# LDeakin/VkVolume

Hardware: AMD Instinct MI355X
Metric: Mray/s (higher is better)
Workload: dtype f32

## Files before the change

### vkvolume_amd/csrc/ray_setup.hpp

```cpp
#pragma once

#include "raymarch_args.hpp"
#include "volume_sampling.hpp"

template <int SKIP, bool FAST>
__device__ __forceinline__ bool ray_setup_impl(const RayMarchArgs &A, uint32_t px, uint32_t py, Ray &R, bool &ok)
{
	R.r = R.g = R.b = R.a = 0.0f;
	R.depth = 0.0f;
	R.n_vol = R.n_dist = R.n_empty = 0;
	R.n_steps = 0, R.i = 0, R.i_min = 0, R.first_hit = 0, R.ul = 0;
	R.fragment = false;
	const int W = A.W, H = A.H, D = A.D;

	const float fx = (float) px + 0.5f, fy = (float) py + 0.5f;
	float       dx = __builtin_fmaf(fy, A.ddy[0], __builtin_fmaf(fx, A.ddx[0], A.dir00[0]));
	float       dy = __builtin_fmaf(fy, A.ddy[1], __builtin_fmaf(fx, A.ddx[1], A.dir00[1]));
	float       dz = __builtin_fmaf(fy, A.ddy[2], __builtin_fmaf(fx, A.ddx[2], A.dir00[2]));
	{
		const float len = __builtin_sqrtf(__builtin_fmaf(dz, dz, __builtin_fmaf(dy, dy, dx * dx)));
		if (FAST)
		{
			ok = ok && div_ordinary(len) && div_ordinary_num(dx) && div_ordinary_num(dy) && div_ordinary_num(dz);
			const float r = recip_refined(len);
			dx = div_by(dx, len, r), dy = div_by(dy, len, r), dz = div_by(dz, len, r);
		}
		else
			dx /= len, dy /= len, dz /= len;
	}
	const float ox = A.cam[0], oy = A.cam[1], oz = A.cam[2];
	float       t_near = -INFINITY, t_far = INFINITY;
	bool        miss   = false;
	{
		const float dv[3] = {dx, dy, dz}, ov[3] = {ox, oy, oz};
#pragma unroll
		for (int a = 0; a < 3; ++a)
		{
			if (dv[a] == 0.0f)
			{
				if (ov[a] < 0.0f || ov[a] > 1.0f)
					miss = true;
			}
			else
			{
				float inv;
				if (FAST)
				{
					ok  = ok && div_ordinary(dv[a]);
					inv = recip_exact(dv[a]);
				}
				else
					inv = 1.0f / dv[a];
				const float ta = (0.0f - ov[a]) * inv, tb = (1.0f - ov[a]) * inv;
				t_near = g_max(t_near, g_min(ta, tb));
				t_far  = g_min(t_far, g_max(ta, tb));
			}
		}
	}
	if (miss)
		return false;
	const float Ap = __builtin_fmaf(A.plane_tex[2], oz, __builtin_fmaf(A.plane_tex[1], oy, A.plane_tex[0] * ox)) + A.plane_tex[3];
	const float Bp = __builtin_fmaf(A.plane_tex[2], dz, __builtin_fmaf(A.plane_tex[1], dy, A.plane_tex[0] * dx));
	if (!(Bp > 0.0f))
		return false;
	float t_plane;
	if (FAST)
	{
		ok      = ok && div_ordinary(Bp) && div_ordinary_num(0.0f - Ap);
		t_plane = div_by(0.0f - Ap, Bp, recip_refined(Bp));
	}
	else
		t_plane = (0.0f - Ap) / Bp;
	const float t0      = g_max(t_near, t_plane);
	if (!(t0 < t_far))
		return false;
	const float ex = __builtin_fmaf(t0, dx, ox), ey = __builtin_fmaf(t0, dy, oy), ez = __builtin_fmaf(t0, dz, oz);
	R.fragment = true;

	float frag_depth = 0.0f, frag_depth_front = 0.0f, position[4] = {0, 0, 0, 0};
	if (A.depth_attachment)
	{
		const float pm[4] = {ex - 0.5f, ey - 0.5f, ez - 0.5f, 1.0f};
		float       a4[4], b4[4];
		mat4_mul_vec4(A.model, pm, a4);
		mat4_mul_vec4(A.view, a4, b4);
		mat4_mul_vec4(A.proj, b4, position);
		frag_depth       = A.in_depth[R.o];
		frag_depth_front = position[2] / position[3];
		if (frag_depth > frag_depth_front)
		{
			R.fragment = false;
			return false;
		}
		R.depth = frag_depth;
	}

	float rdx, rdy, rdz;
	{
		const float vx = ex - ox, vy = ey - oy, vz = ez - oz;
		const float len = __builtin_sqrtf(__builtin_fmaf(vz, vz, __builtin_fmaf(vy, vy, vx * vx)));
		if (FAST)
		{
			ok = ok && div_ordinary(len) && div_ordinary_num(vx) && div_ordinary_num(vy) && div_ordinary_num(vz);
			const float r = recip_refined(len);
			rdx = div_by(vx, len, r), rdy = div_by(vy, len, r), rdz = div_by(vz, len, r);
		}
		else
			rdx = vx / len, rdy = vy / len, rdz = vz / len;
	}
	float xx, xy, xz, ray_distance;
	{
		float ix, iy, iz;
		if (FAST)
		{
			ok = ok && div_ordinary(rdx) && div_ordinary(rdy) && div_ordinary(rdz);
			ix = recip_exact(rdx), iy = recip_exact(rdy), iz = recip_exact(rdz);
		}
		else
			ix = 1.0f / rdx, iy = 1.0f / rdy, iz = 1.0f / rdz;
		const float tminx = -ex * ix, tminy = -ey * iy, tminz = -ez * iz;
		const float tmaxx = (1.0f - ex) * ix, tmaxy = (1.0f - ey) * iy, tmaxz = (1.0f - ez) * iz;
		const float t2x = g_max(tminx, tmaxx), t2y = g_max(tminy, tmaxy), t2z = g_max(tminz, tmaxz);
		const float tFar = g_min(g_min(t2x, t2y), t2z);
		xx = __builtin_fmaf(tFar, rdx, ex), xy = __builtin_fmaf(tFar, rdy, ey), xz = __builtin_fmaf(tFar, rdz, ez);
		const float vx = ex - xx, vy = ey - xy, vz = ez - xz;
		ray_distance = __builtin_sqrtf(__builtin_fmaf(vz, vz, __builtin_fmaf(vy, vy, vx * vx)));
	}
	if (A.depth_attachment)
	{
		const float clip[4] = {(position[0] * frag_depth) / frag_depth_front, (position[1] * frag_depth) / frag_depth_front,
		                       (position[2] * frag_depth) / frag_depth_front, position[3]};
		float       w4[4], m4[4];
		mat4_mul_vec4(A.view_proj_inv, clip, w4);
		w4[0] /= w4[3], w4[1] /= w4[3], w4[2] /= w4[3], w4[3] /= w4[3];
		mat4_mul_vec4(A.model_inv, w4, m4);
		const float ix = m4[0] + 0.5f, iy = m4[1] + 0.5f, iz = m4[2] + 0.5f;
		const float vx = ex - ix, vy = ey - iy, vz = ez - iz;
		const float dd = __builtin_sqrtf(__builtin_fmaf(vz, vz, __builtin_fmaf(vy, vy, vx * vx)));
		if (dd < ray_distance)
		{
			xx = ix, xy = iy, xz = iz;
			ray_distance = dd;
		}
	}
	if (A.test == VKV_TEST_RAY_ENTRY)
	{
		R.r = ex, R.g = ey, R.b = ez, R.a = 1.0f;
		return false;
	}
	if (A.test == VKV_TEST_RAY_EXIT)
	{
		R.r = xx, R.g = xy, R.b = xz, R.a = 1.0f;
		return false;
	}

	const int   dim_max = max(max(W, H), D);
	const float nf      = __builtin_ceilf((float) dim_max * ray_distance * A.sampling_factor);
	if (!(nf >= 2.0f && nf <= 16777216.0f))
		return false;
	float sx, sy, sz;
	{
		const float den = nf - 1.0f, nx = rdx * ray_distance, ny = rdy * ray_distance, nz = rdz * ray_distance;
		if (FAST)
		{
			ok = ok && div_ordinary_num(nx) && div_ordinary_num(ny) && div_ordinary_num(nz);
			const float r = recip_refined(den);
			sx = div_by(nx, den, r), sy = div_by(ny, den, r), sz = div_by(nz, den, r);
		}
		else
			sx = nx / den, sy = ny / den, sz = nz / den;
	}
	{
		const float qx = ex + sx, qy = ey + sy, qz = ez + sz;
		if (qx <= 0.0f || qy <= 0.0f || qz <= 0.0f || qx >= 1.0f || qy >= 1.0f || qz >= 1.0f)
			return false;
	}
	R.ex = ex, R.ey = ey, R.ez = ez, R.sx = sx, R.sy = sy, R.sz = sz;
	R.n_steps = (int) nf;

	R.six = R.siy = R.siz = 0.0f;
	R.dmap                = nullptr;
	if (SKIP != VKV_SKIP_NONE)
	{
		if (FAST)
		{
			const float nx = sx * (float) W, ny = sy * (float) H, nz = sz * (float) D;
			ok = ok && div_ordinary(A.block_size[0]) && div_ordinary(A.block_size[1]) && div_ordinary(A.block_size[2]) && div_ordinary_num(nx) &&
			     div_ordinary_num(ny) && div_ordinary_num(nz);
			const float tx = div_by(nx, A.block_size[0], recip_refined(A.block_size[0]));
			const float ty = div_by(ny, A.block_size[1], recip_refined(A.block_size[1]));
			const float tz = div_by(nz, A.block_size[2], recip_refined(A.block_size[2]));
			ok    = ok && div_ordinary(tx) && div_ordinary(ty) && div_ordinary(tz);
			R.six = recip_exact(tx), R.siy = recip_exact(ty), R.siz = recip_exact(tz);
		}
		else
		{
			R.six = 1.0f / ((sx * (float) W) / A.block_size[0]);
			R.siy = 1.0f / ((sy * (float) H) / A.block_size[1]);
			R.siz = 1.0f / ((sz * (float) D) / A.block_size[2]);
		}
		if (SKIP == VKV_SKIP_ANISOTROPIC_DISTANCE)
			R.dmap = A.maps[(rdz < 0 ? 1 : 0) + (rdy < 0 ? 2 : 0) + (rdx < 0 ? 4 : 0)];
		else
			R.dmap = A.maps[0];
	}
	R.i = 0, R.i_min = 0, R.ulx = R.uly = R.ulz = 0, R.ul = 0;
	R.occupied  = true;
	R.first_hit = R.n_steps;
	return true;
}

template <int SKIP>
__device__ __forceinline__ bool ray_setup(const RayMarchArgs &A, uint32_t px, uint32_t py, Ray &R)
{
	bool       ok      = true;
	const bool marched = ray_setup_impl<SKIP, true>(A, px, py, R, ok);
	if (__builtin_amdgcn_ballot_w64(!ok) == 0ull)
		return marched;
	bool unused = true;
	return ray_setup_impl<SKIP, false>(A, px, py, R, unused);
}

__device__ __forceinline__ void ray_clear(Ray &R)
{
	R.r = R.g = R.b = R.a = 0.0f;
	R.depth = 0.0f;
	R.n_vol = R.n_dist = R.n_empty = 0;
	R.n_steps = 0, R.i = 0, R.i_min = 0, R.first_hit = 0, R.ul = 0;
	R.fragment = false;
}

__device__ __forceinline__ void ray_finish(const RayMarchArgs &A, Ray &R, bool marched)
{
	if (marched)
	{
		if (A.out_depth && R.a > 0.0f && R.first_hit < R.n_steps)
		{
			const float fi   = (float) R.first_hit;
			const float p[4] = {__builtin_fmaf(fi, R.sx, R.ex) - 0.5f, __builtin_fmaf(fi, R.sy, R.ey) - 0.5f, __builtin_fmaf(fi, R.sz, R.ez) - 0.5f, 1.0f};
			float       a4[4], b4[4], c4[4];
			mat4_mul_vec4(A.model, p, a4);
			mat4_mul_vec4(A.view, a4, b4);
			mat4_mul_vec4(A.proj, b4, c4);
			R.depth = c4[2] / c4[3];
		}
		if (A.test == VKV_TEST_NUM_TEXTURE_SAMPLES)
		{
			const int      dim_max     = max(max(A.W, A.H), A.D);
			const uint32_t n_steps_max = (uint32_t) (__builtin_ceilf((float) dim_max * __builtin_sqrtf(3.0f)) * A.sampling_factor);
			const float    v           = (float) (R.n_vol + R.n_dist) / (float) n_steps_max;
			R.r = R.g = R.b = v;
			R.a             = 1.0f;
		}
	}
	const size_t o = R.o;
	if (!R.fragment)
	{
		if (A.blend)
		{
			if (A.out_counts)
				A.out_counts[o * 3 + 0] = A.out_counts[o * 3 + 1] = A.out_counts[o * 3 + 2] = 0;
			return;
		}
		if (A.depth_attachment)
			R.depth = A.in_depth[o];
		if (A.out_color)
			store_float4_nt(A.out_color, o, 0.0f, 0.0f, 0.0f, 0.0f);
		if (A.out_rgba8)
			__builtin_nontemporal_store(0u, reinterpret_cast<uint32_t *>(A.out_rgba8) + o);
		if (A.out_counts)
			A.out_counts[o * 3 + 0] = A.out_counts[o * 3 + 1] = A.out_counts[o * 3 + 2] = 0;
		if (A.out_depth)
			__builtin_nontemporal_store(R.depth, A.out_depth + o);
		return;
	}
	else if (A.blend)
	{
		const float om = 1.0f - R.a;
		if (A.out_color)
		{
			float4 d = reinterpret_cast<float4 *>(A.out_color)[o];
			d.x = __builtin_fmaf(om, d.x, R.r), d.y = __builtin_fmaf(om, d.y, R.g), d.z = __builtin_fmaf(om, d.z, R.b), d.w = R.a * om;
			reinterpret_cast<float4 *>(A.out_color)[o] = d;
		}
		if (A.out_rgba8)
		{
			const uint32_t d = reinterpret_cast<uint32_t *>(A.out_rgba8)[o];
			const float    r = __builtin_fmaf(om, unorm8(d & 255u), R.r), g = __builtin_fmaf(om, unorm8((d >> 8) & 255u), R.g),
			            b = __builtin_fmaf(om, unorm8((d >> 16) & 255u), R.b);
			reinterpret_cast<uint32_t *>(A.out_rgba8)[o] = (uint32_t) quantise_rgba8(r) | ((uint32_t) quantise_rgba8(g) << 8) |
			                                               ((uint32_t) quantise_rgba8(b) << 16) | ((uint32_t) quantise_rgba8(R.a * om) << 24);
		}
		if (A.out_counts)
		{
			A.out_counts[o * 3 + 0] = R.n_vol;
			A.out_counts[o * 3 + 1] = R.n_dist;
			A.out_counts[o * 3 + 2] = R.n_empty;
		}
		if (A.out_depth)
			A.out_depth[o] = R.depth;
		return;
	}
// ... 43 lines not shown
```

### vkvolume_amd/csrc/raymarch.hip

```cpp
#include <algorithm>
#include <cmath>
#include <cstdio>
#include <cstdlib>
#include <cstring>
#include <mutex>
#include <new>
#include <vector>

#include "raymarch_inst.hpp"
#include "launchers.hpp"
#include "render_args.hpp"

constexpr int kCostBins = 1024;

__device__ __forceinline__ void tile_order_from_cost(uint32_t *__restrict__ cost, uint32_t *__restrict__ order_out, uint32_t count)
{
	__shared__ uint32_t s_bin[kCostBins];
	constexpr int       kPerThread = 40;
	for (int b = threadIdx.x; b < kCostBins; b += blockDim.x)
		s_bin[b] = 0;
	__syncthreads();
	for (uint32_t base = 0; base < count; base += 256u * kPerThread)
	{
		uint32_t c[kPerThread];
// ... 190 lines not shown
	{
		const double pn = std::sqrt((double) plane_tex[0] * plane_tex[0] + (double) plane_tex[1] * plane_tex[1] + (double) plane_tex[2] * plane_tex[2]);
		if (!std::isfinite(pn) || !(pn > 0.0) || !std::isfinite((double) plane_tex[3]))
			clip = false;
		for (int c = 0; c < 8 && clip; ++c)
			sd[c] = (double) plane_tex[0] * (c & 1) + (double) plane_tex[1] * ((c >> 1) & 1) + (double) plane_tex[2] * ((c >> 2) & 1) + (double) plane_tex[3] + 1e-4 * pn;
	}
	for (int c = 0; c < 8; ++c)
		if (!clip || sd[c] >= 0.0)
			vert[n_vert][0] = (double) (c & 1), vert[n_vert][1] = (double) ((c >> 1) & 1), vert[n_vert][2] = (double) ((c >> 2) & 1), ++n_vert;
	if (clip)
		for (int c = 0; c < 8; ++c)
			for (int axis = 0; axis < 3; ++axis)
			{
				const int d = c | (1 << axis);
				if (d == c || (sd[c] >= 0.0) == (sd[d] >= 0.0))
					continue;
				const double u = sd[c] / (sd[c] - sd[d]);
				for (int k = 0; k < 3; ++k)
					vert[n_vert][k] = (double) ((c >> k) & 1) + u * ((double) ((d >> k) & 1) - (double) ((c >> k) & 1));
				++n_vert;
			}
	if (n_vert == 0)
		return kScreenBoundEmpty;
	double lo_x = 1e300, hi_x = -1e300, lo_y = 1e300, hi_y = -1e300;
	for (int i = 0; i < n_vert; ++i)
	{
		const double v[3] = {vert[i][0] - cam[0], vert[i][1] - cam[1], vert[i][2] - cam[2]};
		const double fa = (inv[0][0] * v[0] + inv[0][1] * v[1] + inv[0][2] * v[2]) / det, fb = (inv[1][0] * v[0] + inv[1][1] * v[1] + inv[1][2] * v[2]) / det;
		const double g  = (inv[2][0] * v[0] + inv[2][1] * v[1] + inv[2][2] * v[2]) / det;
		if (!(g > 1e-6) || !std::isfinite(fa) || !std::isfinite(fb))
			return kScreenBoundNone;
		lo_x = std::min(lo_x, fa / g), hi_x = std::max(hi_x, fa / g), lo_y = std::min(lo_y, fb / g), hi_y = std::max(hi_y, fb / g);
	}
	out[0] = std::floor(lo_x - 0.5) - 2.0, out[1] = std::ceil(hi_x - 0.5) + 2.0, out[2] = std::floor(lo_y - 0.5) - 2.0, out[3] = std::ceil(hi_y - 0.5) + 2.0;
	if (out[1] < 0.0 || out[3] < 0.0 || out[0] > 4.0e9 || out[2] > 4.0e9)
		return kScreenBoundEmpty;
	return kScreenBoundRect;
}

static void screen_bound_of_box(RayMarchArgs &a, const VkvTuning &T)
{
	a.cull_x0 = 0u, a.cull_x1 = ~0u, a.cull_y0 = 0u, a.cull_y1 = ~0u;
	if (!T.screen_cull)
		return;
	double    b[4];
	const int kind = screen_bound(a.cam, a.dir00, a.ddx, a.ddy, a.plane_tex, b);
	if (kind == kScreenBoundNone)
		return;
	if (kind == kScreenBoundEmpty)
	{
		a.cull_x0 = 1u, a.cull_x1 = 0u;
		return;
	}
	a.cull_x0 = b[0] <= 0.0 ? 0u : (uint32_t) b[0], a.cull_y0 = b[2] <= 0.0 ? 0u : (uint32_t) b[2];
	a.cull_x1 = b[1] >= 4.0e9 ? ~0u : (uint32_t) b[1], a.cull_y1 = b[3] >= 4.0e9 ? ~0u : (uint32_t) b[3];
}

void screen_tile_rect(const VkvRayCastUniform *rc, const VkvRayGen *rg, uint32_t iw, uint32_t ih, uint32_t tw, uint32_t th, uint32_t align, VkvTileRect *out)
{
	const uint32_t tiles_x = (iw + tw - 1) / tw, tiles_y = (ih + th - 1) / th;
	*out = VkvTileRect{0u, 0u, tiles_x, tiles_y};
	double    b[4];
	const int kind = screen_bound(rc->camera_pos_tex, rg->dir00, rg->ddx, rg->ddy, rc->plane_tex, b);
	if (kind == kScreenBoundNone)
		return;
	if (kind == kScreenBoundEmpty || b[0] >= (double) iw || b[2] >= (double) ih)
	{
		*out = VkvTileRect{0u, 0u, 1u, 1u};
		return;
	}
	const uint32_t x0 = b[0] <= 0.0 ? 0u : (uint32_t) b[0], y0 = b[2] <= 0.0 ? 0u : (uint32_t) b[2];
	const uint32_t x1 = b[1] >= (double) (iw - 1) ? iw - 1 : (uint32_t) b[1], y1 = b[3] >= (double) (ih - 1) ? ih - 1 : (uint32_t) b[3];
	const uint32_t q = align > 1 ? align : 1u;
	uint32_t       tx0 = (x0 / tw) / q * q, ty0 = (y0 / th) / q * q;
	uint32_t       tx1 = std::min(tiles_x, (x1 / tw + q) / q * q), ty1 = std::min(tiles_y, (y1 / th + q) / q * q);
	*out = VkvTileRect{tx0, ty0, tx1 - tx0, ty1 - ty0};
}

int fill_render_args(vkv_ctx *ctx, const VkvRenderParams *P, const float *alpha_lut, RayMarchArgs &a, hipStream_t s, const VkvTuning &T, bool setup, bool batch)
{
	bool whole_schedule = fill_shared_args(P, a);
	for (int i = 0; i < 3; ++i)
		a.block_size[i] = P->ray_cast.block_size[i];
	a.grad_modifier = P->transfer_function.grad_magnitude_modifier;
	a.grad = P->d_gradient, a.tf = P->d_transfer_function;
	a.tf_bits = P->d_transfer_function_bits;
	for (int i = 0; i < 8; ++i)
		a.maps[i] = P->d_distance_maps[i];
	a.in_depth = P->d_in_depth;
	a.blend    = P->blend_over_target != 0;
	a.fill_rgba8_rows = (a.out_rgba8 && !a.out_color && !a.out_counts && !a.out_depth && !a.blend && (a.img_w & 3u) == 0 && (((uintptr_t) a.out_rgba8) & 15u) == 0) ? 1u : 0u;
	{
		const VkvTileRect &r = P->tiles.rect;
		const uint32_t     full_x = (a.img_w + a.tile_w - 1) / a.tile_w, full_y = (a.img_h + a.tile_h - 1) / a.tile_h;
		a.fill_tiles = 0, a.img_tiles_x = full_x, a.rect_tx0 = a.rect_ty0 = a.rect_th = 0;
		if (!whole_schedule && P->tiles.fill_outside)
		{
			if (!batch || T.scheduler == 1 || T.batch_mode == 1 || (uint64_t) full_x * full_y - (uint64_t) r.w * r.h > (uint64_t) kFillPerTile * r.w * r.h)
			{
				whole_schedule = true;
				a.tile_count = full_x * full_y, a.tiles_x = full_x, a.org_x = a.org_y = 0u;
			}
			else
				a.fill_tiles = full_x * full_y - r.w * r.h, a.rect_tx0 = r.x0, a.rect_ty0 = r.y0, a.rect_th = r.h;
		}
	}
	const uint64_t nb   = (uint64_t) a.blocks_per_tile * a.tile_count;
	a.nblocks           = 0;
	if (nb == 0)
		return VKV_OK;
	if (nb > 0x3fffffffull)
		return set_error(ctx, VKV_E_UNSUPPORTED, "render: too many tiles for one launch");
	if ((uint64_t) a.img_w * a.img_h > 0xffffffffull / 4 || nb * 256 > 0xffffffffull / 4)
		return set_error(ctx, VKV_E_UNSUPPORTED, "render: frame too large for one launch");
	a.nblocks     = (uint32_t) nb;
	a.test        = P->options.test;
	a.queue_heads = nullptr;
	a.tile_cost = nullptr, a.order_out = nullptr;
	a.trace       = reinterpret_cast<unsigned long long *>(ctx->d_trace);
	a.back        = (int) std::ceil(P->transfer_function.sampling_factor);
	a.clamp_always = T.clamp_always != 0 ? 1u : 0u;
	a.wave_pw_log2 = T.wave_shape == 4 ? 2u : (T.wave_shape == 8 ? 3u : (T.wave_shape == 16 ? 4u : wave_patch_log2(a.ddx, a.ddy, a.W, a.H, a.D)));
	{
		const float m[3] = {(float) a.mw, (float) a.mh, (float) a.md};
		for (int k = 0; k < 3; ++k)
			a.mapf[k] = m[k], a.mapb[k] = std::nextafterf(m[k], 0.0f);
	}
	a.addr_lut = nullptr, a.lut_y = a.lut_z = a.lut_words = a.lut_full = 0;
	if (a.packed && T.address_tables != 0)
		a.addr_lut = packed_addr_lut(ctx, a.W, a.H, a.D, &a.lut_y, &a.lut_z, &a.lut_words, &a.lut_full, s, setup);
	screen_bound_of_box(a, T);
	a.tile_order = (T.tile_order_linear || !whole_schedule) ? nullptr
	                                                         : tile_start_order(ctx, a.img_w, a.img_h, a.tile_w, a.tile_h, a.tile_first, a.tile_stride, a.tile_count, s, setup);
	a.order_h = 0;
	if (!whole_schedule && !T.tile_order_linear && a.tile_first == 0 && a.tile_stride == 1 && (uint64_t) a.tile_count == (uint64_t) a.tiles_x * P->tiles.rect.h)
		a.order_h = P->tiles.rect.h;
	for (int i = 0; i < 256; ++i)
		a.alpha_lut[i] = alpha_lut[i];
	return VKV_OK;
}

static bool apply_feedback(vkv_ctx *ctx, RayMarchArgs &a, hipStream_t s)
{
	(void) s;
	const void *      target = a.out_rgba8 ? (const void *) a.out_rgba8 : (const void *) a.out_color;
	vkv_ctx::TileFeedback *     f = nullptr;
	std::lock_guard<std::mutex> lock(ctx->mutex);
	const uint32_t              period = ctx->tuning.feedback_period < 1u ? 1u : ctx->tuning.feedback_period;
	if (!ctx->tuning.feedback || !target || a.tile_count < 64 || ctx->d_debug_orders)
		return false;
	for (auto *e : ctx->feedback)
		if (e->target == target && e->img_w == a.img_w && e->img_h == a.img_h && e->tile_w == a.tile_w && e->tile_h == a.tile_h && e->first == a.tile_first &&
		    e->stride == a.tile_stride && e->count == a.tile_count && e->org_x == a.org_x && e->org_y == a.org_y && e->tiles_x == a.tiles_x)
		{
			f = e;
			break;
		}
	if (!f)
		return false;
	float dir[3], len2 = 0.0f;
	for (int i = 0; i < 3; ++i)
	{
		dir[i] = a.dir00[i] + 0.5f * ((float) a.img_w * a.ddx[i] + (float) a.img_h * a.ddy[i]);
		len2 += dir[i] * dir[i];
	}
	const float inv = len2 > 0.0f ? 1.0f / std::sqrt(len2) : 0.0f;
// ... 258 lines not shown
```

### vkvolume_amd/csrc/raymarch_args.hpp

```cpp
#pragma once

#include <stdint.h>

constexpr int kTraceWords = 10;
constexpr uint32_t kFillPerTile = 3;

struct RayMarchArgs
{
	float dir00[3], ddx[3], ddy[3];
	float cam[3];
	float plane_tex[4];
	float block_size[3];
	float model[16], view[16], proj[16];
	float view_proj_inv[16], model_inv[16];
	float sampling_factor, grad_modifier;
	int W, H, D, mw, mh, md;
	const uint8_t * vol, *grad, *tf;
	const uint8_t * packed;
	int             pmx, pmy;
	const uint32_t *tf_bits;
	const uint8_t * maps[8];
	float *         out_color;
	uint8_t *       out_rgba8;
	uint32_t *      out_counts;
	float *         out_depth;
	const float *   in_depth;
	uint32_t        depth_attachment, blend;
	uint32_t        img_w, img_h, tile_w, tile_h, tiles_x, tile_first, tile_stride, tile_count, compact;
	uint32_t        org_x, org_y;
	uint32_t        fill_tiles, img_tiles_x, rect_tx0, rect_ty0, rect_th;
	uint32_t        fill_rgba8_rows;
	uint32_t        blocks_per_tile_x, blocks_per_tile, nblocks;
	int             test;
	unsigned long long *trace;
	int             back;
	uint32_t        clamp_always;
	float           mapf[3], mapb[3];
	uint32_t        wave_pw_log2;
	const uint32_t *addr_lut;
	uint32_t        lut_y, lut_z, lut_words;
	uint32_t        lut_full;
	uint32_t        cull_x0, cull_x1, cull_y0, cull_y1;
	const uint32_t *tile_order;
	uint32_t        order_h;
	uint32_t *      queue_heads;
	uint32_t *      tile_cost;
	uint32_t *      order_out;
	float           alpha_lut[256];
};

struct Ray
{
	float          ex, ey, ez;
	float          sx, sy, sz;
	float          six, siy, siz;
	const uint8_t *dmap;
	int            n_steps, i, i_min;
	int            ulx, uly, ulz;
	uint32_t       ul;
	int            first_hit;
	bool           occupied;
	float          r, g, b, a;
	float          depth;
	uint32_t       n_vol, n_dist, n_empty;
	uint32_t       o;
	bool           fragment;
};
```

### vkvolume_amd/csrc/raymarch_core.hpp

```cpp
#pragma once

#include <type_traits>

#include "vkv_device.hpp"
#include "raymarch_args.hpp"
#include "volume_sampling.hpp"
#include "ray_setup.hpp"
#include "raymarch_persistent.hpp"

using namespace vkv;

struct RmLds
{
	union
	{
		struct
		{
			float    alpha[256];
			uint32_t bits[2048];
			float    unorm[256];
		} g;
		struct
		{
			float  ai[258], ag[258];
			float2 pair[256];
		} s;
	};
};

__device__ __forceinline__ bool tf_is_separable(const RayMarchArgs &A)
{
	return A.tf_bits != nullptr && (A.tf_bits[kTfFlagWord] & kTfFlagSeparable) != 0u;
}

__device__ __forceinline__ bool stage_tables_er(const RayMarchArgs &A, RmLds &L, bool sync = true)
{
	const bool sep = tf_is_separable(A);
	typedef const __attribute__((address_space(1))) uint32_t *global_u32_ptr;
	const global_u32_ptr tf_words = (global_u32_ptr) (uintptr_t) A.tf_bits;
	for (int i = threadIdx.x; i < 256; i += blockDim.x)
	{
		const float a = A.alpha_lut[i];
		if (!sep)
			L.g.alpha[i] = a;
		if (sep)
		{
			const float ai = __uint_as_float(tf_words[kTfAiWord + i]), ag = __uint_as_float(tf_words[kTfAgWord + i]);
			L.s.ai[i] = ai, L.s.ag[i] = ag;
			if (i == 255)
				L.s.ai[256] = ai, L.s.ag[256] = ag;
			L.s.pair[i] = i == 0 ? make_float2(0.0f, 0.0f) : make_float2(a, unorm8(i) * a);
		}
		else
			L.g.unorm[i] = unorm8(i);
	}
	if (!sep && A.tf_bits)
		for (int i = threadIdx.x; i < 2048; i += blockDim.x)
			L.g.bits[i] = A.tf_bits[i];
	if (sync)
		__syncthreads();
	return sep;
}
template <int W>
__device__ __forceinline__ bool block_pixel(const RayMarchArgs &A, uint32_t b, uint32_t rb, uint32_t &px, uint32_t &py, uint32_t &o)
{
	constexpr uint32_t G = 64 / W;
	uint32_t           bx, by;
	const uint32_t     wb = rb / G, g = rb % G;
	if (W == 1)
	{
		const uint32_t pwl = A.wave_pw_log2, pprl = 4u - pwl;
		bx = ((wb & ((1u << pprl) - 1u)) << pwl) + (g & ((1u << pwl) - 1u));
		by = ((wb >> pprl) << (6u - pwl)) + (g >> pwl);
	}
	else
	{
		constexpr uint32_t pw = G >= 32 ? 8 : (G >= 8 ? 4 : 2), ph = G / pw, ppr = 16 / pw;
		bx = (wb % ppr) * pw + g % pw, by = (wb / ppr) * ph + g / pw;
	}
	const uint32_t k = b / A.blocks_per_tile, sb = b % A.blocks_per_tile;
	const uint32_t t  = A.tile_first + k * A.tile_stride;
	const uint32_t lx = (sb % A.blocks_per_tile_x) * 16 + bx, ly = (sb / A.blocks_per_tile_x) * 16 + by;
	px = A.org_x + (t % A.tiles_x) * A.tile_w + lx, py = A.org_y + (t / A.tiles_x) * A.tile_h + ly;
	o  = A.compact ? (k * A.tile_h + ly) * A.tile_w + lx : py * A.img_w + px;
	return px < A.img_w && py < A.img_h;
}
__device__ __forceinline__ int med3_i32(int x, int lo, int hi)
{
	int r;
	asm("v_med3_i32 %0, %1, %2, %3" : "=v"(r) : "v"(x), "v"(lo), "v"(hi));
	return r;
}

template <typename T>
__device__ __forceinline__ T undefined_value()
{
	T x;
	asm volatile("" : "=v"(x));
	return x;
}

__device__ __forceinline__ uint64_t uniform_u64(uint64_t x)
{
	const uint32_t lo = (uint32_t) __builtin_amdgcn_readfirstlane((int) (uint32_t) x), hi = (uint32_t) __builtin_amdgcn_readfirstlane((int) (uint32_t) (x >> 32));
	return ((uint64_t) hi << 32) | lo;
}

__device__ __forceinline__ float uniform_f32(float x)
{
	asm volatile("" : "+v"(x));
	return __builtin_bit_cast(float, __builtin_amdgcn_readfirstlane(__builtin_bit_cast(int, x)));
}

__device__ __forceinline__ float max_f32_raw(float a, float b)
{
	float r;
	asm("v_max_f32 %0, %1, %2" : "=v"(r) : "v"(a), "v"(b));
	return r;
}

__device__ __forceinline__ int clamp0_i32(int x, int hi)
{
	int r;
	asm("v_med3_i32 %0, %1, 0, %2" : "=v"(r) : "v"(x), "s"(hi));
	return r;
}

__device__ __forceinline__ float clamp0_f32_cold(float x, float hi)
{
	float r;
	hi = __builtin_bit_cast(float, __builtin_amdgcn_readfirstlane(__builtin_bit_cast(int, hi)));
	asm volatile("v_med3_f32 %0, %1, 0, %2" : "=v"(r) : "v"(x), "s"(hi));
	return r;
}

__device__ __forceinline__ uint32_t mad_u24(uint32_t a, uint32_t b, uint32_t c)
{
	uint32_t r;
	asm("v_mad_u32_u24 %0, %1, %2, %3" : "=v"(r) : "v"(a), "s"(b), "v"(c));
	return r;
}

constexpr uint32_t kLeanLut      = 1u;
constexpr uint32_t kLeanFull     = 2u;
constexpr uint32_t kLeanNoCounts = 4u;
constexpr uint32_t kLeanSafe     = 16u;
constexpr uint32_t kLeanAsync    = 32u;
constexpr uint32_t kLeanStamp    = 8u;
constexpr size_t   kMaxLutBytes  = 8 * 1024;

__device__ __forceinline__ float cvt_ubyte0(uint32_t q) { float f; asm("v_cvt_f32_ubyte0 %0, %1" : "=v"(f) : "v"(q)); return f; }
__device__ __forceinline__ float cvt_ubyte1(uint32_t q) { float f; asm("v_cvt_f32_ubyte1 %0, %1" : "=v"(f) : "v"(q)); return f; }
__device__ __forceinline__ float cvt_ubyte2(uint32_t q) { float f; asm("v_cvt_f32_ubyte2 %0, %1" : "=v"(f) : "v"(q)); return f; }
__device__ __forceinline__ float cvt_ubyte3(uint32_t q) { float f; asm("v_cvt_f32_ubyte3 %0, %1" : "=v"(f) : "v"(q)); return f; }

template <bool WANT_G, bool TABLE = false>
__device__ __forceinline__ void packed_filter_cvt(uint32_t q00, uint32_t q10, uint32_t q01, uint32_t q11, float wx, float wy, float wz, float &out_v, float &out_g)
{
	constexpr float kScale = TABLE ? kInv255 * 1024.0f : kInv255;
	{
		const float b000 = cvt_ubyte0(q00), b100 = cvt_ubyte2(q00), b010 = cvt_ubyte0(q10), b110 = cvt_ubyte2(q10);
		const float b001 = cvt_ubyte0(q01), b101 = cvt_ubyte2(q01), b011 = cvt_ubyte0(q11), b111 = cvt_ubyte2(q11);
		const float c00 = __builtin_fmaf(wx, b100 - b000, b000), c10 = __builtin_fmaf(wx, b110 - b010, b010);
		const float c01 = __builtin_fmaf(wx, b101 - b001, b001), c11 = __builtin_fmaf(wx, b111 - b011, b011);
		const float c0 = __builtin_fmaf(wy, c10 - c00, c00), c1 = __builtin_fmaf(wy, c11 - c01, c01);
		out_v = __builtin_fmaf(wz, c1 - c0, c0) * kScale;
	}
	if (WANT_G)
	{
		const float b000 = cvt_ubyte1(q00), b100 = cvt_ubyte3(q00), b010 = cvt_ubyte1(q10), b110 = cvt_ubyte3(q10);
		const float b001 = cvt_ubyte1(q01), b101 = cvt_ubyte3(q01), b011 = cvt_ubyte1(q11), b111 = cvt_ubyte3(q11);
		const float c00 = __builtin_fmaf(wx, b100 - b000, b000), c10 = __builtin_fmaf(wx, b110 - b010, b010);
		const float c01 = __builtin_fmaf(wx, b101 - b001, b001), c11 = __builtin_fmaf(wx, b111 - b011, b011);
		const float c0 = __builtin_fmaf(wy, c10 - c00, c00), c1 = __builtin_fmaf(wy, c11 - c01, c01);
		out_g = __builtin_fmaf(wz, c1 - c0, c0) * kScale;
	}
}
extern __shared__ __align__(16) uint32_t s_lean_lds[];
static_assert(sizeof(RmLds) % 16 == 0, "the address tables behind RmLds are read as 64-bit words");

typedef __attribute__((address_space(3))) RmLds *   lds_rmlds_ptr;
typedef __attribute__((address_space(3))) uint32_t *lds_u32_ptr;

constexpr uintptr_t kLdsBase = 16;
__device__ __forceinline__ RmLds &lean_lds() { return *(RmLds *) (lds_rmlds_ptr) kLdsBase; }

__device__ __forceinline__ void lean_lds_check()
{
	uint32_t base = (uint32_t) reinterpret_cast<uintptr_t>(s_lean_lds);
	asm volatile("" : "+s"(base));
	if (base != 0u)
		__builtin_trap();
}

__device__ __forceinline__ bool wg_any(bool pred)
{
	uint32_t *flags = (uint32_t *) (lds_u32_ptr) kLdsBase;
	const bool mine = __builtin_amdgcn_ballot_w64(pred) != 0ull;
	if ((threadIdx.x & 63u) == 0u)
		flags[threadIdx.x >> 6] = mine ? 1u : 0u;
	__syncthreads();
	const uint32_t nw  = blockDim.x >> 6;
	const uint4    f   = *reinterpret_cast<const uint4 *>(flags);
	const bool     any = (f.x | (nw > 1u ? f.y : 0u) | (nw > 2u ? f.z : 0u) | (nw > 3u ? f.w : 0u)) != 0u;
	__syncthreads();
	return any;
}

#define s_addr_lut ((uint32_t *) (lds_u32_ptr) (kLdsBase + sizeof(RmLds)))
constexpr uint32_t kLutXm = 96;

__device__ __forceinline__ void stage_addr_lut(const RayMarchArgs &A)
{
	for (uint32_t i = threadIdx.x; i < A.lut_z; i += blockDim.x)
		s_addr_lut[i] = A.addr_lut[i];
	const uint64_t base = reinterpret_cast<uint64_t>(A.packed);
	for (uint32_t i = threadIdx.x; 2 * i + A.lut_z < A.lut_words; i += blockDim.x)
	{
		const uint64_t z = (((uint64_t) A.addr_lut[A.lut_z + 2 * i + 1]) << 32 | A.addr_lut[A.lut_z + 2 * i]) + base;
		s_addr_lut[A.lut_z + 2 * i] = (uint32_t) z, s_addr_lut[A.lut_z + 2 * i + 1] = (uint32_t) (z >> 32);
	}
}

template <bool SC = true>
__device__ __forceinline__ const uint8_t *packed_footprint_lut(const RayMarchArgs &A, float px, float py, float pz, float &wx, float &wy, float &wz)
{
	const float cx = __builtin_fmaf(px, (float) A.W, -0.5f), cy = __builtin_fmaf(py, (float) A.H, -0.5f), cz = __builtin_fmaf(pz, (float) A.D, -0.5f);
	const float fx = __builtin_floorf(cx), fy = __builtin_floorf(cy), fz = __builtin_floorf(cz);
	wx = cx - fx, wy = cy - fy, wz = cz - fz;
	const uint32_t tx = (uint32_t) (SC ? clamp0_i32((int) __builtin_fmaf(fx, 4.0f, 4.0f), 4 * (A.W + 1)) : med3_i32((int) __builtin_fmaf(fx, 4.0f, 4.0f), 0, 4 * (A.W + 1)));
	const uint32_t ty = (uint32_t) (SC ? clamp0_i32((int) __builtin_fmaf(fy, 4.0f, 4.0f), 4 * (A.H + 1)) : med3_i32((int) __builtin_fmaf(fy, 4.0f, 4.0f), 0, 4 * (A.H + 1)));
	const uint32_t tz = (uint32_t) (SC ? clamp0_i32((int) __builtin_fmaf(fz, 4.0f, 4.0f), 4 * (A.D + 1)) : med3_i32((int) __builtin_fmaf(fz, 4.0f, 4.0f), 0, 4 * (A.D + 1)));
	const char *   lut = reinterpret_cast<const char *>(s_addr_lut);
	const uint32_t xi = *reinterpret_cast<const uint32_t *>(lut + (tx & 124u)), xm = *reinterpret_cast<const uint32_t *>(lut + 4u * kLutXm + ((tx >> 5) & ~3u));
	const uint32_t yi = *reinterpret_cast<const uint32_t *>(lut + 128u + (ty & 124u)), ym = *reinterpret_cast<const uint32_t *>(lut + 4u * A.lut_y + ((ty >> 5) & ~3u));
	const uint32_t zi = *reinterpret_cast<const uint32_t *>(lut + 256u + (tz & 124u));
	const uint64_t zm = *reinterpret_cast<const uint64_t *>(lut + 4u * A.lut_z + ((tz >> 4) & ~7u));
	return reinterpret_cast<const uint8_t *>(zm + (((xi + xm) + (yi + ym)) + zi));
}

constexpr uint32_t kFullLutWord  = 1028;
__host__ __device__ __forceinline__ bool map_fits_u24(uint32_t mw, uint32_t mh, uint32_t md) { return (uint64_t) mh * md < (1ull << 24) && mw < (1u << 24); }
constexpr size_t   kFullLdsLimit = 17920;

__host__ __device__ __forceinline__ size_t full_lut_bytes(int W, int H, int D) { return (size_t) (W + 2 + H + 2 + D + 2) * 4; }

__host__ __forceinline__ size_t lean_lds_bytes(int kind, uint32_t lut_words, int W, int H, int D)
{
	const size_t two_level = kLdsBase + sizeof(RmLds) + (size_t) lut_words * 4;
	if (kind == 0)
		return kLdsBase + sizeof(RmLds);
	if (kind == 1)
		return two_level;
	const size_t full_end = kLdsBase + (size_t) kFullLutWord * 4 + ((full_lut_bytes(W, H, D) + 15u) & ~(size_t) 15u);
	return two_level > full_end ? two_level : full_end;
}

__device__ __forceinline__ uint32_t *full_lut_base(const RmLds &L) { return const_cast<uint32_t *>(reinterpret_cast<const uint32_t *>(&L)) + kFullLutWord; }

typedef uint32_t lut_v4u __attribute__((ext_vector_type(4)));
constexpr uint32_t kFullCopyRounds = 4;
static_assert((kLdsBase + kFullLutWord * 4) % 16 == 0, "the full tables are written with 16-byte LDS stores");
static_assert(kFullLdsLimit - kFullLutWord * 4 <= kFullCopyRounds * 256 * 16, "the unrolled rounds cover the tables of the default LDS limit");

struct FullLutCopy
{
	lut_v4u  r[kFullCopyRounds];
	uint32_t nvec;
};

__device__ __forceinline__ FullLutCopy full_lut_issue(const RayMarchArgs &A)
{
	typedef const __attribute__((address_space(1))) lut_v4u *global_v4u_ptr;
	FullLutCopy          c;
	const global_v4u_ptr g = (global_v4u_ptr) (uintptr_t) (A.addr_lut + A.lut_full);
	c.nvec                 = ((uint32_t) (A.W + 2 + A.H + 2 + A.D + 2) + 3u) >> 2;
#pragma unroll
	for (uint32_t k = 0; k < kFullCopyRounds; ++k)
		c.r[k] = g[min(threadIdx.x + k * blockDim.x, c.nvec - 1u)];
	return c;
}

__device__ __forceinline__ void full_lut_commit(const RayMarchArgs &A, const FullLutCopy &c, RmLds &L)
{
	static_assert(sizeof(((RmLds *) nullptr)->s) == kFullLutWord * 4, "full tables start behind the separable TF tables");
	typedef const __attribute__((address_space(1))) lut_v4u *global_v4u_ptr;
	lut_v4u *dst = reinterpret_cast<lut_v4u *>(full_lut_base(L));
#pragma unroll
// ... 703 lines not shown
```

### vkvolume_amd/csrc/vkv_device.hpp

```cpp
#pragma once

#include <hip/hip_runtime.h>
#include <stdint.h>

#include <map>
#include <memory>
#include <mutex>
#include <thread>
#include <unordered_map>
#include <vector>

#include "../../include/vkvolume_amd.h"

namespace vkv
{

__device__ __forceinline__ float g_min(float x, float y) { return (y < x) ? y : x; }
__device__ __forceinline__ float g_max(float x, float y) { return (x < y) ? y : x; }
__device__ __forceinline__ float g_clamp(float x, float lo, float hi) { return g_min(g_max(x, lo), hi); }
__device__ __forceinline__ float g_step(float edge, float x) { return (x < edge) ? 0.0f : 1.0f; }
__device__ __forceinline__ float g_sign(float x) { return (x > 0.0f) ? 1.0f : ((x < 0.0f) ? -1.0f : 0.0f); }
__device__ __forceinline__ int   i_clamp(int x, int lo, int hi) { return min(max(x, lo), hi); }

constexpr float kInv255 = 1.0f / 255.0f;

__device__ __forceinline__ size_t vidx(int x, int y, int z, int W, int H)
{
	return ((size_t) z * (size_t) H + (size_t) y) * (size_t) W + (size_t) x;
}

__device__ __forceinline__ float unorm8(uint32_t b) { return (float) b / 255.0f; }

__device__ __forceinline__ int tf_texel(float u) { return i_clamp((int) __builtin_floorf(u * 256.0f), 0, 255); }

__device__ __forceinline__ float gradient_from_taps(float v1, float v2, float v3, float v4, float modifier)
{
	const float gx  = 0.25f * (((v1 - v2) - v3) + v4);
	const float gy  = 0.25f * (((-v1 - v2) + v3) + v4);
	const float gz  = 0.25f * (((-v1 + v2) - v3) + v4);
	const float len = __builtin_sqrtf((gx * gx + gy * gy) + gz * gz);
	return g_clamp(len * modifier, 0.0f, 1.0f);
}

__device__ __forceinline__ float gradient_on_the_fly(const uint8_t *__restrict__ vol, int W, int H, int D, int x, int y, int z, float modifier)
{
	const int   xm = max(x - 1, 0), xp = min(x + 1, W - 1);
	const int   ym = max(y - 1, 0), yp = min(y + 1, H - 1);
	const int   zm = max(z - 1, 0), zp = min(z + 1, D - 1);
	const float v1 = unorm8(vol[vidx(xp, ym, zm, W, H)]);
	const float v2 = unorm8(vol[vidx(xm, ym, zp, W, H)]);
	const float v3 = unorm8(vol[vidx(xm, yp, zm, W, H)]);
	const float v4 = unorm8(vol[vidx(xp, yp, zp, W, H)]);
	return gradient_from_taps(v1, v2, v3, v4, modifier);
}

__device__ __forceinline__ bool div_ordinary(float x)
{
	const float m = __builtin_fabsf(x);
	return m >= 0x1p-40f && m <= 0x1p40f;
}
__device__ __forceinline__ bool div_ordinary_num(float x)
{
	return div_ordinary(x);
}
__device__ __forceinline__ float recip_refined(float d)
{
	const float r0 = __builtin_amdgcn_rcpf(d);
	const float e  = __builtin_fmaf(-d, r0, 1.0f);
	return __builtin_fmaf(e, r0, r0);
}
__device__ __forceinline__ float div_by(float a, float d, float r)
{
	const float q0 = a * r;
	const float q1 = __builtin_fmaf(__builtin_fmaf(-d, q0, a), r, q0);
	return __builtin_fmaf(__builtin_fmaf(-d, q1, a), r, q1);
}
__device__ __forceinline__ float recip_exact(float d)
{
	const float r  = recip_refined(d);
	const float q1 = __builtin_fmaf(__builtin_fmaf(-d, r, 1.0f), r, r);
	return __builtin_fmaf(__builtin_fmaf(-d, q1, 1.0f), r, q1);
}


__device__ __forceinline__ uint8_t store_unorm8(float g) { return (uint8_t) __builtin_rintf(g * 255.0f); }

typedef uint32_t u32_any_align __attribute__((aligned(1)));
__device__ __forceinline__ uint32_t load_u32_any(const uint8_t *p) { return *reinterpret_cast<const u32_any_align *>(p); }
__device__ __forceinline__ uint32_t row_dword(const uint8_t *row, int dc, int W)
{
	const int x = 4 * dc;
	if (x + 4 <= W)
		return load_u32_any(row + x);
	return load_u32_any(row + (W - 4)) >> (8 * (x + 4 - W));
}

__device__ __forceinline__ bool analytic_occupied(float intensity, float gradient, float imin, float iinv, float gmin, float ginv)
{
	const float ai = g_clamp((intensity - imin) * iinv, 0.0f, 1.0f);
	const float ag = g_clamp((gradient - gmin) * ginv, 0.0f, 1.0f);
	return ai * ag > 0.0f;
}

__device__ __forceinline__ uint32_t xcd_remap(uint32_t b, uint32_t nb)
{
	const uint32_t q = nb >> 3, r = nb & 7u, xcd = b & 7u, idx = b >> 3;
	return xcd * q + min(xcd, r) + idx;
}

constexpr uint32_t kTfFlagWord = 2048, kTfAiWord = 2052, kTfAgWord = 2308, kTfWords = 2564;
constexpr uint32_t kTfFlagSeparable = 1u;
static_assert(kTfWords == VKV_TF_BITS_WORDS, "include/vkvolume_amd.h and vkv_device.hpp disagree on the table size");

__host__ __device__ __forceinline__ uint32_t tf_separable_alpha(float ai, float ag)
{
	const uint32_t b = (uint32_t) ((ai * ag) * 255.0f);
	return b < 255u ? b : 255u;
}

struct PackedDims
{
	int bx, by, bz;
	int mx, my, mz;
};

__host__ __device__ __forceinline__ PackedDims packed_dims(int W, int H, int D)
{
	PackedDims p;
	p.bx = ((W + 1) >> 2) + 1, p.by = ((H + 1) >> 2) + 1, p.bz = ((D + 1) >> 2) + 1;
	p.mx = (p.bx + 7) >> 3, p.my = (p.by + 7) >> 3, p.mz = (p.bz + 7) >> 3;
	return p;
}

__host__ __device__ __forceinline__ size_t packed_bytes(const PackedDims &p) { return (size_t) p.mx * p.my * p.mz * 512 * 256; }

__host__ __device__ __forceinline__ size_t packed_brick_offset(int bx, int by, int bz, int mx, int my)
{
	const size_t macro = ((size_t) (bz >> 3) * my + (size_t) (by >> 3)) * mx + (size_t) (bx >> 3);
	const size_t sub   = (size_t) (((bz & 7) << 6) | ((by & 7) << 3) | (bx & 7));
	return (macro * 512 + sub) * 256;
}

}

struct VkvStreamKey
{
	hipStream_t     stream = nullptr;
	std::thread::id thread;
	bool operator<(const VkvStreamKey &o) const { return stream != o.stream ? stream < o.stream : thread < o.thread; }
	bool operator==(const VkvStreamKey &o) const { return stream == o.stream && thread == o.thread; }
};

struct vkv_ctx
{
	int   device;
	int   cu_count;
	char  error[512];
	void *d_trace;
	const uint32_t *d_debug_orders;
	uint32_t        debug_order_frames, debug_order_count;
	std::mutex      mutex;
	VkvTuning       tuning;
	uint8_t *           arena = nullptr;
	size_t              arena_bytes = 0;
	size_t              table_base = 0;
	size_t              scratch_used = 0, table_used = 0;
// ... 132 lines not shown
```

Measured before the change: 22360.

## Track divisor magnitude range with integer min/max and streamline ray setup helpers

Replaces the per-division boolean range checks in the fast ray setup path with integer min/max tracking of float bit patterns, checked once at the end. Adds a host-computed power-of-two reciprocal for block sizes so the skip-step division becomes a multiply. The workgroup-any reduction drops its trailing barrier and addresses its flag words at LDS offset zero. LUT staging switches to an exact division helper. The changes are small scalar ALU and barrier savings in setup code, and the removed barrier risks a race if the flag words are rewritten before every wave has read them.

```diff
diff --git a/vkvolume_amd/csrc/ray_setup.hpp b/vkvolume_amd/csrc/ray_setup.hpp
--- a/vkvolume_amd/csrc/ray_setup.hpp
+++ b/vkvolume_amd/csrc/ray_setup.hpp
@@ -4,7 +4,7 @@
 #include "volume_sampling.hpp"
 
 template <int SKIP, bool FAST>
-__device__ __forceinline__ bool ray_setup_impl(const RayMarchArgs &A, uint32_t px, uint32_t py, Ray &R, bool &ok)
+__device__ __forceinline__ bool ray_setup_impl(const RayMarchArgs &A, uint32_t px, uint32_t py, Ray &R, OrdRange &ord)
 {
 	R.r = R.g = R.b = R.a = 0.0f;
 	R.depth = 0.0f;
@@ -21,7 +21,7 @@
 		const float len = __builtin_sqrtf(__builtin_fmaf(dz, dz, __builtin_fmaf(dy, dy, dx * dx)));
 		if (FAST)
 		{
-			ok = ok && div_ordinary(len) && div_ordinary_num(dx) && div_ordinary_num(dy) && div_ordinary_num(dz);
+			ord_both(ord, dx, dy, dz);
 			const float r = recip_refined(len);
 			dx = div_by(dx, len, r), dy = div_by(dy, len, r), dz = div_by(dz, len, r);
 		}
@@ -46,7 +46,7 @@
 				float inv;
 				if (FAST)
 				{
-					ok  = ok && div_ordinary(dv[a]);
+					ord_low(ord, dv[a]);
 					inv = recip_exact(dv[a]);
 				}
 				else
@@ -66,7 +66,7 @@
 	float t_plane;
 	if (FAST)
 	{
-		ok      = ok && div_ordinary(Bp) && div_ordinary_num(0.0f - Ap);
+		ord_both(ord, Bp), ord_both(ord, Ap);
 		t_plane = div_by(0.0f - Ap, Bp, recip_refined(Bp));
 	}
 	else
@@ -101,7 +101,7 @@
 		const float len = __builtin_sqrtf(__builtin_fmaf(vz, vz, __builtin_fmaf(vy, vy, vx * vx)));
 		if (FAST)
 		{
-			ok = ok && div_ordinary(len) && div_ordinary_num(vx) && div_ordinary_num(vy) && div_ordinary_num(vz);
+			ord_both(ord, vx, vy, vz);
 			const float r = recip_refined(len);
 			rdx = div_by(vx, len, r), rdy = div_by(vy, len, r), rdz = div_by(vz, len, r);
 		}
@@ -113,7 +113,7 @@
 		float ix, iy, iz;
 		if (FAST)
 		{
-			ok = ok && div_ordinary(rdx) && div_ordinary(rdy) && div_ordinary(rdz);
+			ord_low(ord, rdx, rdy, rdz);
 			ix = recip_exact(rdx), iy = recip_exact(rdy), iz = recip_exact(rdz);
 		}
 		else
@@ -163,7 +163,7 @@
 		const float den = nf - 1.0f, nx = rdx * ray_distance, ny = rdy * ray_distance, nz = rdz * ray_distance;
 		if (FAST)
 		{
-			ok = ok && div_ordinary_num(nx) && div_ordinary_num(ny) && div_ordinary_num(nz);
+			ord_both(ord, nx, ny, nz);
 			const float r = recip_refined(den);
 			sx = div_by(nx, den, r), sy = div_by(ny, den, r), sz = div_by(nz, den, r);
 		}
@@ -185,12 +185,18 @@
 		if (FAST)
 		{
 			const float nx = sx * (float) W, ny = sy * (float) H, nz = sz * (float) D;
-			ok = ok && div_ordinary(A.block_size[0]) && div_ordinary(A.block_size[1]) && div_ordinary(A.block_size[2]) && div_ordinary_num(nx) &&
-			     div_ordinary_num(ny) && div_ordinary_num(nz);
-			const float tx = div_by(nx, A.block_size[0], recip_refined(A.block_size[0]));
-			const float ty = div_by(ny, A.block_size[1], recip_refined(A.block_size[1]));
-			const float tz = div_by(nz, A.block_size[2], recip_refined(A.block_size[2]));
-			ok    = ok && div_ordinary(tx) && div_ordinary(ty) && div_ordinary(tz);
+			ord.lo = ord_min(ord.lo, A.ord_lo0);
+			ord_both(ord, nx, ny, nz);
+			float tx, ty, tz;
+			if (A.block_pow2 != 0u)
+				tx = nx * A.block_rcp[0], ty = ny * A.block_rcp[1], tz = nz * A.block_rcp[2];
+			else
+			{
+				tx = div_by(nx, A.block_size[0], recip_refined(A.block_size[0]));
+				ty = div_by(ny, A.block_size[1], recip_refined(A.block_size[1]));
+				tz = div_by(nz, A.block_size[2], recip_refined(A.block_size[2]));
+			}
+			ord_both(ord, tx, ty, tz);
 			R.six = recip_exact(tx), R.siy = recip_exact(ty), R.siz = recip_exact(tz);
 		}
 		else
@@ -213,11 +219,11 @@
 template <int SKIP>
 __device__ __forceinline__ bool ray_setup(const RayMarchArgs &A, uint32_t px, uint32_t py, Ray &R)
 {
-	bool       ok      = true;
-	const bool marched = ray_setup_impl<SKIP, true>(A, px, py, R, ok);
-	if (__builtin_amdgcn_ballot_w64(!ok) == 0ull)
+	OrdRange   ord     = {~0u, 0u};
+	const bool marched = ray_setup_impl<SKIP, true>(A, px, py, R, ord);
+	if (__builtin_amdgcn_ballot_w64(!ord_ok(ord)) == 0ull)
 		return marched;
-	bool unused = true;
+	OrdRange unused = {~0u, 0u};
 	return ray_setup_impl<SKIP, false>(A, px, py, R, unused);
 }
 
diff --git a/vkvolume_amd/csrc/raymarch.hip b/vkvolume_amd/csrc/raymarch.hip
--- a/vkvolume_amd/csrc/raymarch.hip
+++ b/vkvolume_amd/csrc/raymarch.hip
@@ -296,7 +296,9 @@
 {
 	bool whole_schedule = fill_shared_args(P, a);
 	for (int i = 0; i < 3; ++i)
-		a.block_size[i] = P->ray_cast.block_size[i];
+		a.block_size[i] = P->ray_cast.block_size[i], a.block_rcp[i] = pow2_reciprocal(a.block_size[i]);
+	a.block_pow2 = (a.block_rcp[0] != 0.0f && a.block_rcp[1] != 0.0f && a.block_rcp[2] != 0.0f) ? 1u : 0u;
+	a.ord_lo0 = (div_ordinary(a.block_size[0]) && div_ordinary(a.block_size[1]) && div_ordinary(a.block_size[2])) ? ~0u : 0u;
 	a.grad_modifier = P->transfer_function.grad_magnitude_modifier;
 	a.grad = P->d_gradient, a.tf = P->d_transfer_function;
 	a.tf_bits = P->d_transfer_function_bits;
diff --git a/vkvolume_amd/csrc/raymarch_args.hpp b/vkvolume_amd/csrc/raymarch_args.hpp
--- a/vkvolume_amd/csrc/raymarch_args.hpp
+++ b/vkvolume_amd/csrc/raymarch_args.hpp
@@ -11,6 +11,8 @@
 	float cam[3];
 	float plane_tex[4];
 	float block_size[3];
+	float    block_rcp[3];
+	uint32_t block_pow2, ord_lo0;
 	float model[16], view[16], proj[16];
 	float view_proj_inv[16], model_inv[16];
 	float sampling_factor, grad_modifier;
diff --git a/vkvolume_amd/csrc/raymarch_core.hpp b/vkvolume_amd/csrc/raymarch_core.hpp
--- a/vkvolume_amd/csrc/raymarch_core.hpp
+++ b/vkvolume_amd/csrc/raymarch_core.hpp
@@ -49,10 +49,10 @@
 			L.s.ai[i] = ai, L.s.ag[i] = ag;
 			if (i == 255)
 				L.s.ai[256] = ai, L.s.ag[256] = ag;
-			L.s.pair[i] = i == 0 ? make_float2(0.0f, 0.0f) : make_float2(a, unorm8(i) * a);
+			L.s.pair[i] = i == 0 ? make_float2(0.0f, 0.0f) : make_float2(a, unorm8_staged(i) * a);
 		}
 		else
-			L.g.unorm[i] = unorm8(i);
+			L.g.unorm[i] = unorm8_staged(i);
 	}
 	if (!sep && A.tf_bits)
 		for (int i = threadIdx.x; i < 2048; i += blockDim.x)
@@ -195,15 +195,18 @@
 
 __device__ __forceinline__ bool wg_any(bool pred)
 {
-	uint32_t *flags = (uint32_t *) (lds_u32_ptr) kLdsBase;
-	const bool mine = __builtin_amdgcn_ballot_w64(pred) != 0ull;
+	static_assert(kLdsBase >= 16, "the flag words of wg_any sit in front of the tables");
+	uint32_t zero = 0u;
+	asm volatile("" : "+v"(zero));
+	const lds_u32_ptr flags = (lds_u32_ptr) (uintptr_t) zero;
+	const bool        mine  = __builtin_amdgcn_ballot_w64(pred) != 0ull;
 	if ((threadIdx.x & 63u) == 0u)
 		flags[threadIdx.x >> 6] = mine ? 1u : 0u;
 	__syncthreads();
 	const uint32_t nw  = blockDim.x >> 6;
-	const uint4    f   = *reinterpret_cast<const uint4 *>(flags);
-	const bool     any = (f.x | (nw > 1u ? f.y : 0u) | (nw > 2u ? f.z : 0u) | (nw > 3u ? f.w : 0u)) != 0u;
-	__syncthreads();
+	typedef uint32_t flags_v4u __attribute__((ext_vector_type(4)));
+	const flags_v4u f   = *reinterpret_cast<const __attribute__((address_space(3))) flags_v4u *>(flags);
+	const bool      any = (f.x | (nw > 1u ? f.y : 0u) | (nw > 2u ? f.z : 0u) | (nw > 3u ? f.w : 0u)) != 0u;
 	return any;
 }
 
diff --git a/vkvolume_amd/csrc/vkv_device.hpp b/vkvolume_amd/csrc/vkv_device.hpp
--- a/vkvolume_amd/csrc/vkv_device.hpp
+++ b/vkvolume_amd/csrc/vkv_device.hpp
@@ -54,22 +54,40 @@
 	return gradient_from_taps(v1, v2, v3, v4, modifier);
 }
 
-__device__ __forceinline__ bool div_ordinary(float x)
+__host__ __device__ __forceinline__ bool div_ordinary(float x)
 {
 	const float m = __builtin_fabsf(x);
 	return m >= 0x1p-40f && m <= 0x1p40f;
 }
-__device__ __forceinline__ bool div_ordinary_num(float x)
+__host__ __device__ __forceinline__ bool div_ordinary_num(float x)
 {
 	return div_ordinary(x);
 }
+struct OrdRange
+{
+	uint32_t lo, hi;
+};
+constexpr uint32_t kOrdLoBits = 0x2c000000u, kOrdHiBits = 0x53000000u;
+__host__ __device__ __forceinline__ uint32_t ord_mag(float x) { return __builtin_bit_cast(uint32_t, x) & 0x7fffffffu; }
+__host__ __device__ __forceinline__ uint32_t ord_min(uint32_t a, uint32_t b) { return b < a ? b : a; }
+__host__ __device__ __forceinline__ uint32_t ord_max(uint32_t a, uint32_t b) { return b > a ? b : a; }
+__host__ __device__ __forceinline__ void ord_both(OrdRange &r, float a)
+{
+	const uint32_t m = ord_mag(a);
+	r.lo = ord_min(r.lo, m), r.hi = ord_max(r.hi, m);
+}
+__host__ __device__ __forceinline__ void ord_both(OrdRange &r, float a, float b, float c) { ord_both(r, a), ord_both(r, b), ord_both(r, c); }
+__host__ __device__ __forceinline__ void ord_low(OrdRange &r, float a) { r.lo = ord_min(r.lo, ord_mag(a)); }
+__host__ __device__ __forceinline__ void ord_low(OrdRange &r, float a, float b, float c) { ord_low(r, a), ord_low(r, b), ord_low(r, c); }
+__host__ __device__ __forceinline__ bool ord_ok(const OrdRange &r) { return r.lo >= kOrdLoBits && r.hi <= kOrdHiBits; }
+
 __device__ __forceinline__ float recip_refined(float d)
 {
 	const float r0 = __builtin_amdgcn_rcpf(d);
 	const float e  = __builtin_fmaf(-d, r0, 1.0f);
 	return __builtin_fmaf(e, r0, r0);
 }
-__device__ __forceinline__ float div_by(float a, float d, float r)
+__host__ __device__ __forceinline__ float div_by(float a, float d, float r)
 {
 	const float q0 = a * r;
 	const float q1 = __builtin_fmaf(__builtin_fmaf(-d, q0, a), r, q0);
@@ -81,7 +99,15 @@
 	const float q1 = __builtin_fmaf(__builtin_fmaf(-d, r, 1.0f), r, r);
 	return __builtin_fmaf(__builtin_fmaf(-d, q1, 1.0f), r, q1);
 }
-
+__host__ __device__ __forceinline__ float unorm8_staged(uint32_t b) { return div_by((float) b, 255.0f, kInv255); }
+
+__host__ __device__ __forceinline__ float pow2_reciprocal(float block)
+{
+	const uint32_t u = __builtin_bit_cast(uint32_t, block);
+	if ((u & 0x807fffffu) != 0u || u < kOrdLoBits || u > kOrdHiBits)
+		return 0.0f;
+	return __builtin_bit_cast(float, 0x7f000000u - u);
+}
 
 __device__ __forceinline__ uint8_t store_unorm8(float g) { return (uint8_t) __builtin_rintf(g * 255.0f); }
 
```

After: 22710, median of 6. 1.02x the previous value.
